# mahfuzalhasan/WaveFormer

Measured on AMD Instinct MI355X. Metric: 128³×4 volumes/sec fwd (1/2/4/8 MI355X) + Dice Δ vs reference, higher is better.
Workload: dtype bf16x3; 1 GPU; MultiscaleTransformer (WaveFormer encoder) forward, 128^3x4 crops; global_batch=8, per_gpu_batch=8, precision=bf16x3, parallelism=replicas x1 (no data-path collective), hip_graph=True

## Files before the change

waveformer_amd/csrc/ffn_dwfc2_tb.hip:

```cpp
#include "ffn_dwfc_common.hpp"

namespace wf {

#ifdef WF_DWFC2_PROBE
__device__ long long g_dwfc2tb_probe[16 * 8];
extern "C" int wf_debug_dwfc2tb_probe(long long* host) {
  return (int)hipMemcpyFromSymbol(host, HIP_SYMBOL(g_dwfc2tb_probe), sizeof(g_dwfc2tb_probe));
}
#endif

namespace tb2 {
constexpr int S2 = 4;
constexpr int C = 96, HID = 384, TY = 4, TX = 4;
constexpr int PY = TY + 2, PX = TX + 2, PP = PY * PX;
constexpr int NPOS = TY * TX;
constexpr int HS = HID + 8, WKP = HID + 8;
constexpr int PLANE_F = PP * HID;
constexpr int H2F = NPOS * HS;
constexpr int NV = HID / 4;
constexpr int NPC = PP * NV / 64;
constexpr int NPCE = (NPC + 3) / 4;
constexpr int KS = HID / 32, KH = KS / 2;
constexpr int NVEC = 2 * HID + 3 * C;
constexpr size_t LDS_BYTES = (size_t)(PLANE_F + H2F + NVEC) * 4 + (size_t)C * WKP * 2 + 2 * 1024 + 16;
static_assert(PP * NV == NPC * 64 && PX * NV == 9 * 64, "whole pieces, 9 per haloed row");
static_assert(LDS_BYTES <= 160 * 1024, "LDS");
static_assert(HID * 28 <= PLANE_F, "depthwise weights and bias staged in the plane buffer");
}

template <int P>
__global__ __launch_bounds__(1024, 1) void ffn_dwfc2_tb_kernel(DwFcArgs a) {
  using namespace tb2;
  constexpr bool SPLIT = P == PREC_SPLIT;
  __shared__ __attribute__((aligned(16))) float plane[PLANE_F];
  __shared__ __attribute__((aligned(16))) float h2t[H2F];
  __shared__ __attribute__((aligned(16))) uint16_t wf[C * WKP];
  __shared__ __attribute__((aligned(16))) float vecs[NVEC];
  __shared__ f32x4 fcpart[2 * 64];
  __shared__ int simd_cnt[4];
  float* lnw = vecs;
  float* lnb = lnw + HID;
  float* fcb = lnb + HID;
  float* n2w = fcb + C;
  float* n2b = n2w + C;

  const int tid = threadIdx.x;
  const int wid = tid >> 6, lane = tid & 63;
  const int D = a.D, H = a.H, W = a.W;
  const DwFcTile tl = dwfc_tile<TY, TX>(a);
  const int b = tl.b, x0 = tl.x0, y0 = tl.y0, z0 = tl.z0, z1 = tl.z1;
  const int plane_sz = H * W;

  if (tid < 4) simd_cnt[tid] = 0;
  for (int i = tid; i < C * (HID / 8); i += 1024) {
    const int n = i / (HID / 8), k8 = i % (HID / 8);
    *reinterpret_cast<bf16x8*>(wf + n * WKP + 8 * k8) =
        *reinterpret_cast<const bf16x8*>(a.fc + (size_t)n * HID + 8 * k8);
  }
  dwfc_stage_ln2<HID>(lnw, lnb, a, 1024);
  dwfc_stage_epi<C>(fcb, n2w, n2b, a, 1024);
  for (int i = tid; i < HID * 27; i += 1024) plane[i] = a.dw_w[i];
  for (int i = tid; i < HID; i += 1024) plane[HID * 27 + i] = a.dw_b[i];
  __syncthreads();
  const int role = dwfc_wave_role<4>(simd_cnt, wid, lane);
  PROBE_DECL
#ifdef WF_DWFC2_PROBE
  pr_acc[6] = role;
#endif

  if (role < 12) {
    const int xp = role / 6, kslot = role % 3, c = (role % 6) * 64 + lane;
    float w[27];
#pragma unroll
    for (int k = 0; k < 27; ++k) w[k] = plane[c * 27 + k];
    const float bias = plane[HID * 27 + c];
    float acc[3][TY][2];
#pragma unroll
    for (int s = 0; s < 3; ++s)
#pragma unroll
      for (int o = 0; o < TY; ++o) acc[s][o][0] = acc[s][o][1] = 0.f;
    const int lpos = 2 * (2 * (role / 3) + kslot) + (lane >> 5), lg = lane & 31;
    const float* q0 = plane + 2 * xp * HID + c;
    const int dbg = ffn_dbg(a);

    auto ln2_rows = [&]() {
      dwfc_ln2_row<P, HID, 32, 128, false>(h2t + lpos * HS, 4 * lg, lnw, lnb, a.eps2);
    };
    auto load_plane = [&](float (&vin)[PY][4]) {
#pragma unroll
      for (int r = 0; r < PY; ++r)
#pragma unroll
        for (int k = 0; k < 4; ++k) vin[r][k] = q0[(r * PX + k) * HID];
    };
    auto rows = [&](const float (&vin)[PY][4], auto SAc, auto SBc, auto SCc, auto LOc, auto HIc) {
      constexpr int SA = decltype(SAc)::value, SB = decltype(SBc)::value,
                    SC = decltype(SCc)::value, LO = decltype(LOc)::value, HI = decltype(HIc)::value;
      if (dbg & 1) return;
#pragma unroll
      for (int r = LO; r < HI; ++r) {
        const float u0 = vin[r][0], u1 = vin[r][1], u2 = vin[r][2], u3 = vin[r][3];
#pragma unroll
        for (int ky = 0; ky < 3; ++ky) {
          const int o = r - ky;
          if (o < 0 || o >= TY) continue;
          const float* w0 = w + ky * 3;
          acc[SC][o][0] = fmaf(w0[2], u2, fmaf(w0[1], u1, fmaf(w0[0], u0, acc[SC][o][0])));
          acc[SC][o][1] = fmaf(w0[2], u3, fmaf(w0[1], u2, fmaf(w0[0], u1, acc[SC][o][1])));
          acc[SB][o][0] = fmaf(w0[11], u2, fmaf(w0[10], u1, fmaf(w0[9], u0, acc[SB][o][0])));
          acc[SB][o][1] = fmaf(w0[11], u3, fmaf(w0[10], u2, fmaf(w0[9], u1, acc[SB][o][1])));
          acc[SA][o][0] = fmaf(w0[20], u2, fmaf(w0[19], u1, fmaf(w0[18], u0, acc[SA][o][0])));
          acc[SA][o][1] = fmaf(w0[20], u3, fmaf(w0[19], u2, fmaf(w0[18], u1, acc[SA][o][1])));
        }
      }
    };
    typedef std::integral_constant<int, 0> I0;
    typedef std::integral_constant<int, 1> I1;
    typedef std::integral_constant<int, 2> I2;
    typedef std::integral_constant<int, S2> IS;
    typedef std::integral_constant<int, PY> IP;
    auto step = [&](int p, auto Rc) {
      constexpr int R = decltype(Rc)::value;
      typedef std::integral_constant<int, (R + 1) % 3> SA;
      typedef std::integral_constant<int, (R + 2) % 3> SB;
      typedef std::integral_constant<int, R> SC;
      const bool valid = p - 1 >= z0, more = p + 1 <= z1;
      __syncthreads();
      PROBE(5)
      if (valid) {
#pragma unroll
        for (int o = 0; o < TY; ++o)
#pragma unroll
          for (int q = 0; q < 2; ++q) h2t[(o * TX + 2 * xp + q) * HS + c] = acc[R][o][q] + bias;
      }
#pragma unroll
      for (int o = 0; o < TY; ++o) acc[R][o][0] = acc[R][o][1] = 0.f;
      PROBE(0)
      __syncthreads();
      PROBE(1)
      float vin[PY][4];
      if (more) load_plane(vin);
      __syncthreads();
      PROBE(7)
      if (kslot < 2) {
        if (valid && !(dbg & 2)) ln2_rows();
      } else if (more) {
        rows(vin, SA(), SB(), SC(), I0(), IS());
      }
      PROBE(2)
      __syncthreads();
      PROBE(3)
      if (more) {
        if (kslot < 2) rows(vin, SA(), SB(), SC(), I0(), IP());
        else rows(vin, SA(), SB(), SC(), IS(), IP());
      }
      PROBE(4)
    };
    __syncthreads();
    __syncthreads();
    {
      float vin[PY][4];
      load_plane(vin);
      __syncthreads();
      rows(vin, I0(), I1(), I2(), I0(), IP());
    }
    for (int p = z0 - 1; p <= z1; p += 3) {
      step(p, I0());
      if (p + 1 <= z1) step(p + 1, I1());
      if (p + 2 <= z1) step(p + 2, I2());
    }
    __syncthreads();
    PROBE_DUMP_TO(g_dwfc2tb_probe)
    return;
  }

  __builtin_amdgcn_s_setprio(3);
  const int e = role - 12;
  const int l15 = lane & 15, g4 = lane >> 4;
  const int pair = e >> 1;
  const bool upper = e & 1;
  const int tf = 3 * pair + (upper ? 2 : 0);
  const int th = 3 * pair + 1;
  const int kh0 = upper ? KH : 0;
  const int colf = tf * 16 + 4 * g4, colh = th * 16 + 4 * g4;
  const float bs = __builtin_bit_cast(
      float, __builtin_amdgcn_readfirstlane(__builtin_bit_cast(int, a.bscale ? a.bscale[b] : 1.f)));
  const int dbg = ffn_dbg(a);
  bf16x8 fwf[KS], fwh[KH];
  {
    const uint16_t* wr = a.fc + (size_t)(C + tf * 16 + l15) * HID + 8 * g4;
    const uint16_t* wh = a.fc + (size_t)(C + th * 16 + l15) * HID + 8 * g4 + kh0 * 32;
#pragma unroll
    for (int ks = 0; ks < KS; ++ks)
      fwf[ks] = SPLIT ? *reinterpret_cast<const bf16x8*>(wr + ks * 32) : bf16x8{0, 0, 0, 0, 0, 0, 0, 0};
#pragma unroll
    for (int ks = 0; ks < KH; ++ks)
      fwh[ks] = SPLIT ? *reinterpret_cast<const bf16x8*>(wh + ks * 32) : bf16x8{0, 0, 0, 0, 0, 0, 0, 0};
  }
  const float* src = reinterpret_cast<const float*>(a.h1) + (int64_t)b * D * plane_sz * HID;
  const int64_t plane_elems = (int64_t)plane_sz * HID;
  auto stage = [&](int p) {
    const bool pz = p >= 0 && p < D && p <= z1 && !(dbg & 8);
    const float* base = src + (int64_t)min(max(p, 0), D - 1) * plane_elems - HID;
    const __amdgpu_buffer_rsrc_t rs = buf_rsrc(base, pz ? (int)((plane_elems + HID) * 4) : 0);
    int ln = lane, es = e;
    asm volatile("" : "+v"(ln), "+s"(es));
    const int l16 = ln * 16, hbit = ln >= 32 ? 2 : 1;
#pragma unroll
    for (int k = 0; k < NPCE; ++k) {
      const int j = min(4 * k + es, NPC - 1);
      const int r = j / 9, q = j - 9 * r, m = q / 3, q3 = q - 3 * m;
      const int yy = y0 - 1 + r;
      const int xlo = x0 - 1 + 2 * m + (q3 == 2), xhi = x0 - 1 + 2 * m + (q3 >= 1);
      const bool rowok = yy >= 0 && yy < H;
      const int okbits = (rowok && xlo >= 0 && xlo < W ? 1 : 0) | (rowok && xhi >= 0 && xhi < W ? 2 : 0);
      const int voff = (okbits & hbit) ? l16 : BUF_OOR;
      const int soff = (max(yy, 0) * W + x0) * (HID * 4) + q * 1024;
      __builtin_amdgcn_raw_ptr_buffer_load_lds(
          rs, (__attribute__((address_space(3))) void*)(plane + j * 256), 16, voff, soff, 0, 0);
    }
  };
  const int yo = y0 + l15 / TX, xo = x0 + l15 % TX;
  const bool rv = yo < H && xo < W;
  const int gpos0 = b * D * plane_sz + min(yo, H - 1) * W + min(xo, W - 1);
  const float* sbase = a.stats ? a.stats : a.x;
  const int64_t npos = (int64_t)a.B * D * plane_sz;
  const __amdgpu_buffer_rsrc_t xrsrc = buf_rsrc(a.x, (int)(npos * C * 4));
  const __amdgpu_buffer_rsrc_t srsrc = buf_rsrc(sbase, (int)(npos * 2 * 4));
  const __amdgpu_buffer_rsrc_t orsrc = buf_rsrc(a.out, (int)(npos * C * 4));
  f32x4 xrf = f32x4{0.f, 0.f, 0.f, 0.f}, xrh = xrf;
  f32x2 esf = f32x2{0.f, 1.f}, esh = esf;
  auto load_resid = [&](int z, int col, bool own, f32x4& xv, f32x2& ev) {
    const int g = gpos0 + min(max(z, 0), D - 1) * plane_sz;
    xv = __builtin_bit_cast(f32x4, __builtin_amdgcn_raw_buffer_load_b128(
                                       xrsrc, own ? (g * C + col) * 4 : BUF_OOR, 0, 0));
    ev = __builtin_bit_cast(f32x2, __builtin_amdgcn_raw_buffer_load_b64(srsrc, own ? g * 8 : BUF_OOR, 0, 0));
  };
  auto epi_store = [&](f32x4 acc, int z, int col, bool ok, const f32x4& xv, const f32x2& ev) {
    const f32x4 v = dwfc_epilogue(acc, fcb, n2w, n2b, col, xv, ev, bs, a.stats != nullptr);
    const int voff = ok ? ((gpos0 + z * plane_sz) * C + col) * 4 : BUF_OOR;
    __builtin_amdgcn_raw_buffer_store_b128(__builtin_bit_cast(u32x4, v), orsrc, voff, 0, 0);
  };
  f32x4 acch = f32x4{0.f, 0.f, 0.f, 0.f};
  auto finish_half = [&](int z) {
    const f32x4 part = fcpart[pair * 64 + lane];
    epi_store(acch + part, z, colh, !upper && rv && z >= z0, xrh, esh);
    load_resid(z + 1, colh, !upper, xrh, esh);
  };
  const uint16_t* Bh = reinterpret_cast<const uint16_t*>(h2t) + (size_t)l15 * (2 * HS) + 8 * g4;
  const uint16_t* Wf = wf + (size_t)(tf * 16 + l15) * WKP + 8 * g4;
  const uint16_t* Wh = wf + (size_t)(th * 16 + l15) * WKP + 8 * g4;
  auto lds8 = [](const uint16_t* q) { return *reinterpret_cast<const bf16x8*>(q); };
  auto fc = [&](f32x4& accf) {
#pragma unroll
    for (int ks = 0; ks < KS; ++ks) {
      {
        const bf16x8 bh = lds8(Bh + ks * 32), bl = lds8(Bh + (SPLIT ? HID : 0) + ks * 32);
        accf = mma3<P>(accf, lds8(Wf + ks * 32), fwf[ks], bh, bl);
      }
      if (ks < KH) {
        const int k = (kh0 + ks) * 32;
        const bf16x8 bh = lds8(Bh + k), bl = lds8(Bh + (SPLIT ? HID : 0) + k);
        acch = mma3<P>(acch, lds8(Wh + k), fwh[ks], bh, bl);
      }
    }
  };

  __syncthreads();
  stage(z0 - 1);
  asm volatile("s_waitcnt vmcnt(0)" ::: "memory");
  __builtin_amdgcn_s_barrier();
  finish_half(z0 - 3);
  asm volatile("s_waitcnt lgkmcnt(0)" ::: "memory");
  __builtin_amdgcn_s_barrier();
  stage(z0);
  asm volatile("" ::: "memory");
  epi_store(acch, z0 - 2, colf, false, xrf, esf);
  load_resid(z0 - 2, colf, true, xrf, esf);
  for (int p = z0 - 1; p <= z1; ++p) {
    const int zo = p - 1;
    const bool valid = zo >= z0;
    __builtin_amdgcn_s_barrier();
    PROBE(5)
    finish_half(zo - 1);
    asm volatile("s_waitcnt vmcnt(6)" ::: "memory");
    asm volatile("s_waitcnt lgkmcnt(0)" ::: "memory");
    PROBE(0)
    __builtin_amdgcn_s_barrier();
    PROBE(1)
    __builtin_amdgcn_s_barrier();
    PROBE(7)
    stage(p + 2);
    asm volatile("" ::: "memory");
    PROBE(2)
    __builtin_amdgcn_s_barrier();
    PROBE(3)
    f32x4 accf = f32x4{0.f, 0.f, 0.f, 0.f};
    acch = accf;
    if (!(dbg & 4)) {
      fc(accf);
      if (upper) fcpart[pair * 64 + lane] = acch;
    }
    asm volatile("" ::: "memory");
    epi_store(accf, zo, colf, rv && valid, xrf, esf);
    load_resid(zo + 1, colf, true, xrf, esf);
    asm volatile("s_waitcnt lgkmcnt(0)" ::: "memory");
    PROBE(4)
  }
  __builtin_amdgcn_s_barrier();
  finish_half(z1 - 1);
  asm volatile("s_waitcnt vmcnt(0)" ::: "memory");
  PROBE_DUMP_TO(g_dwfc2tb_probe)
}

int launch_ffn_dwfc2_tb(const DwFcArgs& g, int prec, hipStream_t s) {
  using namespace tb2;
  if (prec != PREC_SPLIT && prec != PREC_FP16) return fail(WF_E_SHAPE, "ffn_dwfc2_tb: fp32 h1 only");
  if (!ffn_dwfc2_tb_fits(g))
    return fail(WF_E_SHAPE, "ffn_dwfc2_tb: tensor beyond the 2 GiB buffer-offset range");
  const int64_t blocks =
      (int64_t)g.B * cdiv(g.H, TY) * cdiv(g.W, TX) * cdiv(g.D, g.ZS);
  void (*kern)(DwFcArgs) = prec == PREC_SPLIT ? ffn_dwfc2_tb_kernel<PREC_SPLIT>
                                              : ffn_dwfc2_tb_kernel<PREC_FP16>;
  hipLaunchKernelGGL(kern, dim3((unsigned)blocks), dim3(1024), 0, s, g);
  return check_launch("ffn_dwfc2_tb");
}

}
```

Before: 1265 volumes/s.

## Load dwconv inputs straight to registers and double-buffer h2 tiles

The conv waves now load their haloed input columns directly from global memory into registers with buffer loads. Each row's load for the next plane is interleaved into the FMA loop. This replaces the LDS plane staging that the FC waves used to do through buffer_load_lds. The h2 tile becomes double-buffered, so LayerNorm, depthwise conv and FC for different z-planes overlap, and each step drops from four barriers to two. The cost is more register pressure in the conv waves, redundant global loads of halo columns across waves, and a deeper pipeline prologue and epilogue.

```diff
diff --git a/waveformer_amd/csrc/ffn_dwfc2_tb.hip b/waveformer_amd/csrc/ffn_dwfc2_tb.hip
--- a/waveformer_amd/csrc/ffn_dwfc2_tb.hip
+++ b/waveformer_amd/csrc/ffn_dwfc2_tb.hip
@@ -7,33 +7,31 @@
 extern "C" int wf_debug_dwfc2tb_probe(long long* host) {
   return (int)hipMemcpyFromSymbol(host, HIP_SYMBOL(g_dwfc2tb_probe), sizeof(g_dwfc2tb_probe));
 }
+#define PROBE_VMWAIT asm volatile("s_waitcnt vmcnt(20)" ::: "memory"); PROBE(4)
+#else
+#define PROBE_VMWAIT
 #endif
 
 namespace tb2 {
-constexpr int S2 = 4;
+constexpr int S2 = 6;
 constexpr int C = 96, HID = 384, TY = 4, TX = 4;
-constexpr int PY = TY + 2, PX = TX + 2, PP = PY * PX;
+constexpr int PY = TY + 2;
 constexpr int NPOS = TY * TX;
 constexpr int HS = HID + 8, WKP = HID + 8;
-constexpr int PLANE_F = PP * HID;
 constexpr int H2F = NPOS * HS;
-constexpr int NV = HID / 4;
-constexpr int NPC = PP * NV / 64;
-constexpr int NPCE = (NPC + 3) / 4;
 constexpr int KS = HID / 32, KH = KS / 2;
 constexpr int NVEC = 2 * HID + 3 * C;
-constexpr size_t LDS_BYTES = (size_t)(PLANE_F + H2F + NVEC) * 4 + (size_t)C * WKP * 2 + 2 * 1024 + 16;
-static_assert(PP * NV == NPC * 64 && PX * NV == 9 * 64, "whole pieces, 9 per haloed row");
+constexpr size_t LDS_BYTES = (size_t)(2 * H2F + NVEC) * 4 + (size_t)C * WKP * 2 + 2 * 1024 + 16;
 static_assert(LDS_BYTES <= 160 * 1024, "LDS");
-static_assert(HID * 28 <= PLANE_F, "depthwise weights and bias staged in the plane buffer");
+static_assert(HID * 28 <= 2 * H2F, "depthwise weights and bias staged in the h2 tiles");
+static_assert(S2 >= 0 && S2 <= PY, "S2");
 }
 
 template <int P>
 __global__ __launch_bounds__(1024, 1) void ffn_dwfc2_tb_kernel(DwFcArgs a) {
   using namespace tb2;
   constexpr bool SPLIT = P == PREC_SPLIT;
-  __shared__ __attribute__((aligned(16))) float plane[PLANE_F];
-  __shared__ __attribute__((aligned(16))) float h2t[H2F];
+  __shared__ __attribute__((aligned(16))) float h2b[2 * H2F];
   __shared__ __attribute__((aligned(16))) uint16_t wf[C * WKP];
   __shared__ __attribute__((aligned(16))) float vecs[NVEC];
   __shared__ f32x4 fcpart[2 * 64];
@@ -59,58 +57,101 @@
   }
   dwfc_stage_ln2<HID>(lnw, lnb, a, 1024);
   dwfc_stage_epi<C>(fcb, n2w, n2b, a, 1024);
-  for (int i = tid; i < HID * 27; i += 1024) plane[i] = a.dw_w[i];
-  for (int i = tid; i < HID; i += 1024) plane[HID * 27 + i] = a.dw_b[i];
+  for (int i = tid; i < HID * 27; i += 1024) h2b[i] = a.dw_w[i];
+  for (int i = tid; i < HID; i += 1024) h2b[HID * 27 + i] = a.dw_b[i];
   __syncthreads();
   const int role = dwfc_wave_role<4>(simd_cnt, wid, lane);
   PROBE_DECL
 #ifdef WF_DWFC2_PROBE
   pr_acc[6] = role;
+  pr_acc[7] = z1 + 3 - z0;
 #endif
+  auto bar = [&]() {
+    asm volatile("s_waitcnt lgkmcnt(0)" ::: "memory");
+    __builtin_amdgcn_s_barrier();
+    asm volatile("" ::: "memory");
+  };
 
   if (role < 12) {
     const int xp = role / 6, kslot = role % 3, c = (role % 6) * 64 + lane;
     float w[27];
 #pragma unroll
-    for (int k = 0; k < 27; ++k) w[k] = plane[c * 27 + k];
-    const float bias = plane[HID * 27 + c];
+    for (int k = 0; k < 27; ++k) w[k] = h2b[c * 27 + k];
+    const float bias = h2b[HID * 27 + c];
     float acc[3][TY][2];
 #pragma unroll
     for (int s = 0; s < 3; ++s)
 #pragma unroll
       for (int o = 0; o < TY; ++o) acc[s][o][0] = acc[s][o][1] = 0.f;
     const int lpos = 2 * (2 * (role / 3) + kslot) + (lane >> 5), lg = lane & 31;
-    const float* q0 = plane + 2 * xp * HID + c;
     const int dbg = ffn_dbg(a);
 
-    auto ln2_rows = [&]() {
-      dwfc_ln2_row<P, HID, 32, 128, false>(h2t + lpos * HS, 4 * lg, lnw, lnb, a.eps2);
-    };
-    auto load_plane = [&](float (&vin)[PY][4]) {
-#pragma unroll
-      for (int r = 0; r < PY; ++r)
-#pragma unroll
-        for (int k = 0; k < 4; ++k) vin[r][k] = q0[(r * PX + k) * HID];
-    };
-    auto rows = [&](const float (&vin)[PY][4], auto SAc, auto SBc, auto SCc, auto LOc, auto HIc) {
+    const float* src = reinterpret_cast<const float*>(a.h1) + (int64_t)b * D * plane_sz * HID;
+    const int64_t plane_elems = (int64_t)plane_sz * HID;
+    const int plane_bytes = (int)((plane_elems + HID) * 4);
+    const int c4 = 4 * c;
+    int rowoff[PY], okmask = 0;
+#pragma unroll
+    for (int r = 0; r < PY; ++r) {
+      const int yy = y0 - 1 + r;
+      rowoff[r] = (min(max(yy, 0), H - 1) * W + x0 + 2 * xp) * (HID * 4);
+#pragma unroll
+      for (int k = 0; k < 4; ++k) {
+        const int xx = x0 - 1 + 2 * xp + k;
+        if (yy >= 0 && yy < H && xx >= 0 && xx < W) okmask |= 1 << (4 * r + k);
+      }
+    }
+    struct PlaneSel {
+      const float* base;
+      int mk;
+    };
+    auto plane_sel = [&](int p) {
+      PlaneSel s;
+      s.base = src + (int64_t)min(max(p, 0), D - 1) * plane_elems - HID;
+      s.mk = (p >= 0 && p < D && p <= z1 && !(dbg & 8)) ? okmask : 0;
+      asm volatile("" : "+s"(s.mk));
+      return s;
+    };
+    auto load_row = [&](float (&v)[4], int r, const PlaneSel& s) {
+#pragma unroll
+      for (int k = 0; k < 4; ++k) {
+        const int rng = (s.mk >> (4 * r + k)) & 1 ? plane_bytes : 0;
+        v[k] = __builtin_bit_cast(float, __builtin_amdgcn_raw_buffer_load_b32(
+                                             buf_rsrc(s.base, rng), c4, rowoff[r] + k * (HID * 4), 0));
+      }
+    };
+    auto rows = [&](float (&vin)[PY][4], const PlaneSel& nx, auto SAc, auto SBc, auto SCc, auto LOc,
+                    auto HIc) {
       constexpr int SA = decltype(SAc)::value, SB = decltype(SBc)::value,
                     SC = decltype(SCc)::value, LO = decltype(LOc)::value, HI = decltype(HIc)::value;
-      if (dbg & 1) return;
 #pragma unroll
       for (int r = LO; r < HI; ++r) {
-        const float u0 = vin[r][0], u1 = vin[r][1], u2 = vin[r][2], u3 = vin[r][3];
-#pragma unroll
-        for (int ky = 0; ky < 3; ++ky) {
-          const int o = r - ky;
-          if (o < 0 || o >= TY) continue;
-          const float* w0 = w + ky * 3;
-          acc[SC][o][0] = fmaf(w0[2], u2, fmaf(w0[1], u1, fmaf(w0[0], u0, acc[SC][o][0])));
-          acc[SC][o][1] = fmaf(w0[2], u3, fmaf(w0[1], u2, fmaf(w0[0], u1, acc[SC][o][1])));
-          acc[SB][o][0] = fmaf(w0[11], u2, fmaf(w0[10], u1, fmaf(w0[9], u0, acc[SB][o][0])));
-          acc[SB][o][1] = fmaf(w0[11], u3, fmaf(w0[10], u2, fmaf(w0[9], u1, acc[SB][o][1])));
-          acc[SA][o][0] = fmaf(w0[20], u2, fmaf(w0[19], u1, fmaf(w0[18], u0, acc[SA][o][0])));
-          acc[SA][o][1] = fmaf(w0[20], u3, fmaf(w0[19], u2, fmaf(w0[18], u1, acc[SA][o][1])));
+        if (!(dbg & 1)) {
+          const float u0 = vin[r][0], u1 = vin[r][1], u2 = vin[r][2], u3 = vin[r][3];
+#pragma unroll
+          for (int ky = 0; ky < 3; ++ky) {
+            const int o = r - ky;
+            if (o < 0 || o >= TY) continue;
+            const float* w0 = w + ky * 3;
+            acc[SC][o][0] = fmaf(w0[2], u2, fmaf(w0[1], u1, fmaf(w0[0], u0, acc[SC][o][0])));
+            acc[SC][o][1] = fmaf(w0[2], u3, fmaf(w0[1], u2, fmaf(w0[0], u1, acc[SC][o][1])));
+            acc[SB][o][0] = fmaf(w0[11], u2, fmaf(w0[10], u1, fmaf(w0[9], u0, acc[SB][o][0])));
+            acc[SB][o][1] = fmaf(w0[11], u3, fmaf(w0[10], u2, fmaf(w0[9], u1, acc[SB][o][1])));
+            acc[SA][o][0] = fmaf(w0[20], u2, fmaf(w0[19], u1, fmaf(w0[18], u0, acc[SA][o][0])));
+            acc[SA][o][1] = fmaf(w0[20], u3, fmaf(w0[19], u2, fmaf(w0[18], u1, acc[SA][o][1])));
+          }
         }
+#pragma unroll
+        for (int o = 0; o < TY; ++o)
+          if (o <= r && o >= r - 2)
+            asm volatile(""
+                         : "+v"(acc[SA][o][0]), "+v"(acc[SA][o][1]), "+v"(acc[SB][o][0]),
+                           "+v"(acc[SB][o][1]), "+v"(acc[SC][o][0]), "+v"(acc[SC][o][1])
+                         :
+                         : "memory");
+        __builtin_amdgcn_sched_barrier(0);
+        load_row(vin[r], r, nx);
+        __builtin_amdgcn_sched_barrier(0);
       }
     };
     typedef std::integral_constant<int, 0> I0;
@@ -118,15 +159,33 @@
     typedef std::integral_constant<int, 2> I2;
     typedef std::integral_constant<int, S2> IS;
     typedef std::integral_constant<int, PY> IP;
-    auto step = [&](int p, auto Rc) {
+    float vin[PY][4];
+    auto step = [&](int p, auto Rc, auto LNc) {
       constexpr int R = decltype(Rc)::value;
-      typedef std::integral_constant<int, (R + 1) % 3> SA;
-      typedef std::integral_constant<int, (R + 2) % 3> SB;
-      typedef std::integral_constant<int, R> SC;
-      const bool valid = p - 1 >= z0, more = p + 1 <= z1;
-      __syncthreads();
-      PROBE(5)
-      if (valid) {
+      constexpr bool LN = decltype(LNc)::value;
+      typedef std::integral_constant<int, R> SA;
+      typedef std::integral_constant<int, (R + 1) % 3> SB;
+      typedef std::integral_constant<int, (R + 2) % 3> SC;
+      const PlaneSel nx = plane_sel(p + 1);
+      if (LN) {
+        if (p - 2 >= z0 && p - 2 < z1 && !(dbg & 2))
+          dwfc_ln2_row<P, HID, 32, 128, false>(h2b + ((p - 2 - z0) & 1) * H2F + lpos * HS, 4 * lg,
+                                               lnw, lnb, a.eps2);
+      } else {
+        PROBE_VMWAIT
+        rows(vin, nx, SA(), SB(), SC(), I0(), IS());
+      }
+      PROBE(0)
+      bar();
+      PROBE(1)
+      if (LN) {
+        PROBE_VMWAIT
+        rows(vin, nx, SA(), SB(), SC(), I0(), IP());
+      } else {
+        rows(vin, nx, SA(), SB(), SC(), IS(), IP());
+      }
+      if (p - 1 >= z0 && p - 1 < z1) {
+        float* h2t = h2b + ((p - 1 - z0) & 1) * H2F;
 #pragma unroll
         for (int o = 0; o < TY; ++o)
 #pragma unroll
@@ -134,41 +193,26 @@
       }
 #pragma unroll
       for (int o = 0; o < TY; ++o) acc[R][o][0] = acc[R][o][1] = 0.f;
-      PROBE(0)
-      __syncthreads();
-      PROBE(1)
-      float vin[PY][4];
-      if (more) load_plane(vin);
-      __syncthreads();
-      PROBE(7)
-      if (kslot < 2) {
-        if (valid && !(dbg & 2)) ln2_rows();
-      } else if (more) {
-        rows(vin, SA(), SB(), SC(), I0(), IS());
-      }
       PROBE(2)
-      __syncthreads();
+      bar();
       PROBE(3)
-      if (more) {
-        if (kslot < 2) rows(vin, SA(), SB(), SC(), I0(), IP());
-        else rows(vin, SA(), SB(), SC(), IS(), IP());
-      }
-      PROBE(4)
-    };
-    __syncthreads();
+    };
+    auto march = [&](auto LNc) {
+      for (int p = z0 - 1; p <= z1 + 1; p += 3) {
+        step(p, I0(), LNc);
+        if (p + 1 <= z1 + 1) step(p + 1, I1(), LNc);
+        if (p + 2 <= z1 + 1) step(p + 2, I2(), LNc);
+      }
+    };
     __syncthreads();
     {
-      float vin[PY][4];
-      load_plane(vin);
-      __syncthreads();
-      rows(vin, I0(), I1(), I2(), I0(), IP());
+      const PlaneSel first = plane_sel(z0 - 1);
+#pragma unroll
+      for (int r = 0; r < PY; ++r) load_row(vin[r], r, first);
     }
-    for (int p = z0 - 1; p <= z1; p += 3) {
-      step(p, I0());
-      if (p + 1 <= z1) step(p + 1, I1());
-      if (p + 2 <= z1) step(p + 2, I2());
-    }
-    __syncthreads();
+    if (kslot < 2) march(std::true_type());
+    else march(std::false_type());
+    bar();
     PROBE_DUMP_TO(g_dwfc2tb_probe)
     return;
   }
@@ -196,29 +240,6 @@
     for (int ks = 0; ks < KH; ++ks)
       fwh[ks] = SPLIT ? *reinterpret_cast<const bf16x8*>(wh + ks * 32) : bf16x8{0, 0, 0, 0, 0, 0, 0, 0};
   }
-  const float* src = reinterpret_cast<const float*>(a.h1) + (int64_t)b * D * plane_sz * HID;
-  const int64_t plane_elems = (int64_t)plane_sz * HID;
-  auto stage = [&](int p) {
-    const bool pz = p >= 0 && p < D && p <= z1 && !(dbg & 8);
-    const float* base = src + (int64_t)min(max(p, 0), D - 1) * plane_elems - HID;
-    const __amdgpu_buffer_rsrc_t rs = buf_rsrc(base, pz ? (int)((plane_elems + HID) * 4) : 0);
-    int ln = lane, es = e;
-    asm volatile("" : "+v"(ln), "+s"(es));
-    const int l16 = ln * 16, hbit = ln >= 32 ? 2 : 1;
-#pragma unroll
-    for (int k = 0; k < NPCE; ++k) {
-      const int j = min(4 * k + es, NPC - 1);
-      const int r = j / 9, q = j - 9 * r, m = q / 3, q3 = q - 3 * m;
-      const int yy = y0 - 1 + r;
-      const int xlo = x0 - 1 + 2 * m + (q3 == 2), xhi = x0 - 1 + 2 * m + (q3 >= 1);
-      const bool rowok = yy >= 0 && yy < H;
-      const int okbits = (rowok && xlo >= 0 && xlo < W ? 1 : 0) | (rowok && xhi >= 0 && xhi < W ? 2 : 0);
-      const int voff = (okbits & hbit) ? l16 : BUF_OOR;
-      const int soff = (max(yy, 0) * W + x0) * (HID * 4) + q * 1024;
-      __builtin_amdgcn_raw_ptr_buffer_load_lds(
-          rs, (__attribute__((address_space(3))) void*)(plane + j * 256), 16, voff, soff, 0, 0);
-    }
-  };
   const int yo = y0 + l15 / TX, xo = x0 + l15 % TX;
   const bool rv = yo < H && xo < W;
   const int gpos0 = b * D * plane_sz + min(yo, H - 1) * W + min(xo, W - 1);
@@ -246,69 +267,53 @@
     epi_store(acch + part, z, colh, !upper && rv && z >= z0, xrh, esh);
     load_resid(z + 1, colh, !upper, xrh, esh);
   };
-  const uint16_t* Bh = reinterpret_cast<const uint16_t*>(h2t) + (size_t)l15 * (2 * HS) + 8 * g4;
   const uint16_t* Wf = wf + (size_t)(tf * 16 + l15) * WKP + 8 * g4;
   const uint16_t* Wh = wf + (size_t)(th * 16 + l15) * WKP + 8 * g4;
   auto lds8 = [](const uint16_t* q) { return *reinterpret_cast<const bf16x8*>(q); };
-  auto fc = [&](f32x4& accf) {
-#pragma unroll
-    for (int ks = 0; ks < KS; ++ks) {
-      {
-        const bf16x8 bh = lds8(Bh + ks * 32), bl = lds8(Bh + (SPLIT ? HID : 0) + ks * 32);
-        accf = mma3<P>(accf, lds8(Wf + ks * 32), fwf[ks], bh, bl);
-      }
-      if (ks < KH) {
-        const int k = (kh0 + ks) * 32;
-        const bf16x8 bh = lds8(Bh + k), bl = lds8(Bh + (SPLIT ? HID : 0) + k);
-        acch = mma3<P>(acch, lds8(Wh + k), fwh[ks], bh, bl);
-      }
-    }
-  };
-
-  __syncthreads();
-  stage(z0 - 1);
-  asm volatile("s_waitcnt vmcnt(0)" ::: "memory");
-  __builtin_amdgcn_s_barrier();
-  finish_half(z0 - 3);
-  asm volatile("s_waitcnt lgkmcnt(0)" ::: "memory");
-  __builtin_amdgcn_s_barrier();
-  stage(z0);
-  asm volatile("" ::: "memory");
-  epi_store(acch, z0 - 2, colf, false, xrf, esf);
-  load_resid(z0 - 2, colf, true, xrf, esf);
-  for (int p = z0 - 1; p <= z1; ++p) {
-    const int zo = p - 1;
-    const bool valid = zo >= z0;
-    __builtin_amdgcn_s_barrier();
-    PROBE(5)
-    finish_half(zo - 1);
-    asm volatile("s_waitcnt vmcnt(6)" ::: "memory");
-    asm volatile("s_waitcnt lgkmcnt(0)" ::: "memory");
-    PROBE(0)
-    __builtin_amdgcn_s_barrier();
-    PROBE(1)
-    __builtin_amdgcn_s_barrier();
-    PROBE(7)
-    stage(p + 2);
-    asm volatile("" ::: "memory");
-    PROBE(2)
-    __builtin_amdgcn_s_barrier();
-    PROBE(3)
+  auto fc_tile = [&](int z) {
+    const uint16_t* Bh = reinterpret_cast<const uint16_t*>(h2b + ((z - z0) & 1) * H2F) +
+                         (size_t)l15 * (2 * HS) + 8 * g4;
     f32x4 accf = f32x4{0.f, 0.f, 0.f, 0.f};
     acch = accf;
     if (!(dbg & 4)) {
-      fc(accf);
+#pragma unroll
+      for (int ks = 0; ks < KS; ++ks) {
+        {
+          const bf16x8 bh = lds8(Bh + ks * 32), bl = lds8(Bh + (SPLIT ? HID : 0) + ks * 32);
+          accf = mma3<P>(accf, lds8(Wf + ks * 32), fwf[ks], bh, bl);
+        }
+        if (ks < KH) {
+          const int k = (kh0 + ks) * 32;
+          const bf16x8 bh = lds8(Bh + k), bl = lds8(Bh + (SPLIT ? HID : 0) + k);
+          acch = mma3<P>(acch, lds8(Wh + k), fwh[ks], bh, bl);
+        }
+      }
       if (upper) fcpart[pair * 64 + lane] = acch;
     }
     asm volatile("" ::: "memory");
-    epi_store(accf, zo, colf, rv && valid, xrf, esf);
-    load_resid(zo + 1, colf, true, xrf, esf);
-    asm volatile("s_waitcnt lgkmcnt(0)" ::: "memory");
-    PROBE(4)
+    epi_store(accf, z, colf, rv && z >= z0, xrf, esf);
+    load_resid(z + 1, colf, true, xrf, esf);
+  };
+
+#pragma unroll
+  for (int ks = 0; ks < KS; ++ks) asm volatile("" : "+v"(fwf[ks]));
+#pragma unroll
+  for (int ks = 0; ks < KH; ++ks) asm volatile("" : "+v"(fwh[ks]));
+  __syncthreads();
+  for (int p = z0 - 1; p <= z1 + 1; ++p) {
+    const int zo = p - 3;
+    fc_tile(zo);
+    PROBE(0)
+    bar();
+    PROBE(1)
+    finish_half(zo);
+    PROBE(2)
+    bar();
+    PROBE(3)
   }
-  __builtin_amdgcn_s_barrier();
+  fc_tile(z1 - 1);
+  bar();
   finish_half(z1 - 1);
-  asm volatile("s_waitcnt vmcnt(0)" ::: "memory");
   PROBE_DUMP_TO(g_dwfc2tb_probe)
 }
 
```

Result: faster. 1280 volumes/s, median of 6 (+1.2%).
